# nicolas1805961/Cardiac-Segmentation-Optical-flow

Measured on AMD Instinct MI355X. Metric: cine frames/sec (seg+flow) at 256x256, higher is better.
Workload: dtype f16 MFMA hi/lo split, f32 accumulate (f32-class); 1 GPU; BASELINE config 4: joint seg+flow over 256x256x30 cine slices; Generic_UNet(32 base, 6 pools) 4-flip TTA on every frame + SegFlowGaussian(video.yaml) two-chunk ED-anchored recurrence + fused label warp; image=256x256

## Files before the change

### cardiac-segmentation-optical-flow_amd/cineflow/_lib.py

```python
import ctypes
import os

_HERE = os.path.dirname(os.path.abspath(__file__))
LIB_PATH = os.environ.get("CINEFLOW_LIB") or os.path.join(_HERE, "libcineflow_hip.so")


class CineflowLibraryError(RuntimeError):
    pass


class CineflowError(RuntimeError):
    pass


P = ctypes.c_void_p
I = ctypes.c_int
L = ctypes.c_long
F = ctypes.c_float
DBL = ctypes.c_double

SIGNATURES = {
    "cf_warp_bilinear_2d": [P, P, P, I, I, I, I, P],
    "cf_vecint_2d": [P, P, P, I, I, I, I, P],
    "cf_warp_labels_2d": [P, P, P, I, I, I, I, I, P],
# ... 4 lines not shown
    "cf_corr_volume": [P, P, P, I, I, I, I, I, I, P],
    "cf_corr_volume_route": [P, P, I, I, I, I, I],
    "cf_corr_mfma_enable": [I],
    "cf_corr_pyramid": [P, P, P, I, I, I, I, I, P],
    "cf_corr_lookup": [P, P, P, I, I, I, I, I, P],
    "cf_convex_upsample": [P, P, P, I, I, I, I, P],
    "cf_conv2d": [P, I, P, I, P, L, P, P, P, I, I, I, I, I, I, I, I, I, I, I, I, F, P],
    "cf_conv_transpose2d_k2s2": [P, P, P, P, I, I, I, I, I, I, I, P],
    "cf_conv2d_f16s": [P, I, P, I, P, P, P, P, I, I, I, I, I, I, I, I, I, I, I, I, F, P, I, P],
    "cf_conv3d_f16s": [P, I, P, I, P, P, P, I, I, I, I, I, I, I, I, I, I, F, P, I, P],
    "cf_conv3d_f16s_ok": [I, I, I, I, I, I, I, I, I, I, I],
    "cf_conv3d_pw_f16s": [P, P, P, P, I, I, I, I, I, I, I, I, F, P, I, P],
    "cf_conv3d_pw_f16s_ok": [I, I, I, I, I, I, I, I],
    "cf_conv_transpose2d_k2s2_f16s": [P, P, P, P, I, I, I, I, I, I, I, F, P, I, P],
    "cf_group_norm_apply": [P, P, P, P, P, I, I, I, I, F, I, I, P, P],
    "cf_group_norm_coef": [P, P, P, I, I, I, I, F, P, P],
    "cf_norm_head_1x1": [P, P, F, P, P, P, I, I, I, I, P],
    "cf_batch_norm_coef": [P, P, P, P, F, I, I, P, P],
    "cf_coef_apply_ok": [I, I, L],
    "cf_coef_apply": [P, P, I, F, P, I, I, I, P],
    "cf_conv2d_f16s_prenorm_ok": [I, I, I, I, I],
    "cf_conv_stream_enable": [I],
    "cf_conv2d_f16s_route": [I] * 16 + [P],
    "cf_conv2d_f16s_prenorm": [P, I, P, F, P, P, P, I, I, I, I, F, P, I, P],
    "cf_conv_terms": [I],
    "cf_conv_wino_enable": [I],
    "cf_conv2d_wino_ok": [I, I, I, I, I, I, I],
    "cf_conv2d_wino_form": [I, I, I, I, I, I, I],
    "cf_conv2d_wino_mfma": [I, I, I, I, I, I, I],
    "cf_conv2d_wino": [P, I, P, I, P, P, P, P, I, I, I, I, I, I, I, F, P, I, P],
    "cf_conv2d_wino_prenorm": [P, I, P, F, P, P, P, I, I, I, I, F, P, I, P],
    "cf_group_norm_apply_res_norm": [P, P, P, P, P, I, I, I, I, F, I, I, P, P, P, P, P],
    "cf_group_norm": [P, P, P, P, P, I, I, I, I, F, I, I, P, P],
    "cf_group_norm_stats": [P, P, I, I, I, I, P],
    "cf_group_norm_route": [P, P, P, I, I, I, I, P],
    "cf_layer_norm_cf": [P, P, P, P, I, I, I, F, P],
    "cf_attention_cf": [P, L, P, L, P, L, P, I, I, I, I, I, P],
    "cf_attention_cf_masked": [P, L, P, L, P, L, P, I, I, I, I, I, I, P],
    "cf_attention_cf_route": [P, L, I, I],
    "cf_gru_reset_mul": [P, P, P, I, I, I, P],
    "cf_gru_blend": [P, P, P, P, I, I, I, P],
    "cf_binary": [I, P, P, P, L, L, P],
    "cf_count_out_of_range": [P, L, F, P, P],
    "cf_copy_channels": [P, I, I, P, I, I, I, I, I, I, P],
    "cf_coords_grid": [P, I, I, I, P],
    "cf_crop2d": [P, P, I, I, I, I, I, I, I, P],
# ... 113 lines not shown
```

### cardiac-segmentation-optical-flow_amd/cineflow/ops.py

```python
import collections
import contextlib
import ctypes
import math
import os

import numpy as np
import torch

from ._lib import lib, check

ACT = {None: 0, "none": 0, "gelu": 1, "relu": 2, "lrelu": 3, "tanh": 4, "sigmoid": 5}
ACT_COEF = dict(ACT, mish=6)
RES = {None: 0, "none": 0, "before_act": 1, "after_act": 2}
OP = {"add": 0, "sub": 1, "mul": 2}


def _stream():
    return torch.cuda.current_stream().cuda_stream


def _f32(t, name="tensor"):
    if not isinstance(t, torch.Tensor) or not t.is_cuda:
        raise TypeError("%s must be a CUDA/HIP tensor (cineflow has no CPU path)" % name)
    if t.dtype != torch.float32:
# ... 302 lines not shown
    if res is not None:
        assert res.shape == (B, cout, Ho, Wo)
    assert wpk.dtype == torch.float16 and wpk.is_cuda
    if F16S_RANGE_CHECK:
        _range_check(x1, x2)
    ws, ws_ptr, ws_groups = _stats_args(stats_groups, B, x1.device)
    check(lib().cf_conv2d_f16s(_f32(x1), C1, _opt(x2), C2, wpk.data_ptr(), _opt(bias), _opt(res), _f32(out), out.shape[1], out_coff, B, H, W,
                               cout, kh, kw, stride, pad[0], pad[1], ACT[act], float(alpha) * (2.0 ** -wscale),
                               ws_ptr, ws_groups, _stream()), "cf_conv2d_f16s")
    return (out, ws) if stats_groups else out


F16sRoute = collections.namedtuple("F16sRoute", "route tup terms nimg fused part")


def conv2d_f16s_route(x1, cout, kh, kw, stride=1, pad=(0, 0), x2=None, prenorm=False, transposed=False, stats_groups=None):
    B, C1, H, W = x1.shape
    C2 = 0 if x2 is None else x2.shape[1]
    plan = (ctypes.c_int * 15)()
    route = lib().cf_conv2d_f16s_route(B, C1, C2, H, W, cout, kh, kw, stride, pad[0], pad[1], x1.data_ptr() & 15,
                                       0 if x2 is None else x2.data_ptr() & 15, int(prenorm), int(transposed), stats_groups or 0, plan)
    check(min(route, 0), "cf_conv2d_f16s_route")
    return F16sRoute(route, tuple(plan[1:11]), plan[11], plan[12], bool(plan[13]), plan[14])


def pack_conv3d_weight_f16s(w, c1=None):
    cout, cin, kd, kh, kw = w.shape
    assert (kh, kw) == (3, 3) and kd in (1, 3)
    ntap = kd * 9
    nmt = 1 if cout <= 32 else 2 * ((cout + 63) // 64)
    hi, lo, s, nchunk = _scaled_split(w.reshape(cout, cin, ntap), 16, nmt, c1)
    x = torch.stack([hi, lo]).view(2, nmt, 32, nchunk, 2, 8, ntap)
    return x.permute(1, 3, 6, 0, 4, 2, 5).contiguous().view(-1), s


def conv3d_f16s_ok(B, C1, C2, D, H, W, cout, kernel, stride):
    kernel, stride = tuple(kernel), tuple(stride)
    if kernel[1] != kernel[2] or stride[1] != stride[2]:
        return False
    return lib().cf_conv3d_f16s_ok(B, C1, C2, D, H, W, cout, kernel[0], kernel[1], stride[0], stride[1]) == 1


def conv3d_f16s(x1, wpk, wscale, bias, cout, kernel, stride=(1, 1, 1), x2=None, out=None, alpha=1.0, stats_groups=None):
    B, C1, D, H, W = x1.shape
    C2 = 0 if x2 is None else x2.shape[1]
    kd, kh, kw = kernel
# ... 980 lines not shown
```

### cardiac-segmentation-optical-flow_amd/csrc/conv_f16s.hip

```cpp
#include <hip/hip_fp16.h>
#include <stdlib.h>
#include <string.h>
#include <algorithm>

#include "conv.h"
#include "profile.h"

namespace cf {

typedef float f32x16 __attribute__((ext_vector_type(16)));
typedef _Float16 f16x8 __attribute__((ext_vector_type(8)));

CF_CLOCK_DECL(g_clock_f16s)

struct F16sGeom {
    int TW, TH, NIMG;
    int PH, PW;
    int pstep;
    int ostep;
    int tiles_x, tiles_y, bgroups;
    int nchunk;
    int ablate;
    int c1_pad;
    int NQ;
    int PWR, pwh, kx1, kx2;
    unsigned m_tx, m_ty, m_percg, m_phnq, m_nq, m_nrec, m_phpw, m_pw, m_thtw, m_tw;
};

__host__ __device__ inline unsigned f16s_magic(int d) { return d <= 1 ? 0u : (unsigned)((1ull << 32) / (unsigned)d + 1ull); }
__device__ __forceinline__ int fdiv(int n, int d, unsigned m) { return d <= 1 ? n : (int)__umulhi((unsigned)n, m); }

#ifdef CF_F16S_ABLATION_BUILD
__device__ unsigned long long g_f16s_phase[9];
#define F16S_CLK() __builtin_readcyclecounter()
#endif
template <int KH, int KW, int CK, int WM, int NTW, int MAXT, int NW, int VEC, int PRE, int WL, int TERMS>
__global__ void __launch_bounds__(64 * NW, NW == 8 ? 4 : ((NTW <= 2 && MAXT <= 3) ? 4 : 2))
conv_f16s_kernel(const ConvParams p, const F16sGeom g, const _Float16* __restrict__ wpk) {
    constexpr int KHW = KH * KW;
    constexpr int KS = CK / 16;
    constexpr int REC = CK * 4 + 16;
    constexpr int NT_WG = NTW * (NW / WM);
    constexpr int NG = CK / 8;
    constexpr int NSTAGE = 64 * NW;
    (void)NT_WG;
    extern __shared__ __attribute__((aligned(16))) unsigned char lds[];
    CF_CLOCK_BEGIN();

    const int tid = threadIdx.x;
    const int lane = tid & 63, wave = __builtin_amdgcn_readfirstlane(tid >> 6);
#ifdef CF_F16S_ABLATION_BUILD
    const unsigned long long ph_t0 = F16S_CLK();
    unsigned long long ph_t1 = 0, ph_stage = 0, ph_bar = 0, ph_t2 = 0;
#endif
    const int half = lane >> 5, l31 = lane & 31;
    const int cw = wave % NW;
    const int mt = blockIdx.y * WM + (cw % WM);
    const int ngrp = cw / WM;

// ... 147 lines not shown
                if (!((v_mask[t] >> k) & 1u)) continue;
                f16x4 hi, lo;
                float v[4];
#pragma unroll
                for (int j = 0; j < 4; ++j) {
                    v[j] = stg[t][j][k];
                    if (PRE) {
                        v[j] = (v[j] - cm[j]) * ca[j] + cs[j];
                        v[j] = p.in_slope < 0.f ? gelu_as(v[j]) : (v[j] > 0.f ? v[j] : v[j] * p.in_slope);
                        v[j] = valid ? v[j] : 0.f;
                    }
                }
                split4_f16(v[0], v[1], v[2], v[3], hi, lo);
                *reinterpret_cast<f16x4*>(base + k * REC) = hi;
                *reinterpret_cast<f16x4*>(base + k * REC + CK * 2) = lo;
            }
        }
    };

    float stg0[MAXT][8];
    f32x4v stgv[VT][4];
    if (VEC) issue_loads_v(0, stgv);
    else issue_loads(0, stg0);
    int b_rec[NTW];
#pragma unroll
    for (int nt = 0; nt < NTW; ++nt) {
        int pidx = (ngrp * NTW + nt) * 32 + l31;
        int img = fdiv(pidx, g.TH * g.TW, g.m_thtw);
        int q = pidx - img * (g.TH * g.TW);
        int tyy = fdiv(q, g.TW, g.m_tw), txx = q - tyy * g.TW;
        if (img >= g.NIMG) { img = 0; tyy = 0; txx = 0; }
        b_rec[nt] = ((img * g.PH + tyy * g.ostep) * g.PWR + txx * (g.pwh ? 1 : g.ostep)) * REC + half * 16;
    }

    f32x16 acc1[NTW];
#pragma unroll
    for (int nt = 0; nt < NTW; ++nt)
#pragma unroll
        for (int r = 0; r < 16; ++r) acc1[nt][r] = 0.f;

    constexpr int NSTEP = KHW * KS;
    if constexpr (WL) {
        constexpr int G = (KHW == 9) ? 3 : ((KHW == 1) ? NSTEP : 5);
        constexpr int NGRP = NSTEP / G;
        static_assert(NGRP * G == NSTEP, "weight groups must tile the chunk");
        constexpr int WSLOT = WM * G * 2 * 1024;
// ... 299 lines not shown
                double s1 = 0.0, s2 = 0.0;
                for (int j = 0; j < n; ++j) { s1 += red[2 * (tid + j)]; s2 += red[2 * (tid + j) + 1]; }
                double* w = p.gn_ws + 2L * ((long)b0 * p.gn_groups + co / cpg);
                atomicAdd(w, s1);
                atomicAdd(w + 1, s2);
            }
        }
    }
    CF_CLOCK_END(g_clock_f16s);
#ifdef CF_F16S_ABLATION_BUILD
    if (lane == 0 && ph_t1 && (blockIdx.x & 63) == 5) {
        const unsigned long long t3 = F16S_CLK();
        atomicAdd(&g_f16s_phase[0], ph_t1 - ph_t0);
        atomicAdd(&g_f16s_phase[1], (ph_t2 - ph_t1) - ph_stage - ph_bar);
        atomicAdd(&g_f16s_phase[2], ph_stage);
        atomicAdd(&g_f16s_phase[3], ph_bar);
        atomicAdd(&g_f16s_phase[4], t3 - ph_t2);
        atomicAdd(&g_f16s_phase[5], 1ULL);
        atomicAdd(&g_f16s_phase[6], ph_e1 - ph_t2);
        atomicAdd(&g_f16s_phase[7], ph_e2 - ph_e1);
        atomicAdd(&g_f16s_phase[8], t3 - ph_e2);
    }
#endif
}


static thread_local int t_conv_terms = 3;
int conv_terms() { return t_conv_terms; }

#define CF_F16S_SHAPES(X)                                                                                                                \
     \
    X(3, 3, 16, 1, 1, 2, 8, 1, 0, 1) X(3, 3, 16, 1, 1, 2, 8, 1, 1, 1) X(3, 3, 16, 2, 2, 2, 8, 1, 0, 1) X(3, 3, 16, 2, 2, 2, 8, 1, 1, 1)  \
    X(3, 3, 16, 1, 1, 2, 4, 0, 0, 0) X(3, 3, 16, 1, 1, 2, 4, 1, 0, 0) X(3, 3, 16, 1, 1, 2, 4, 1, 1, 0) X(3, 3, 16, 2, 2, 2, 4, 0, 0, 0)  \
    X(3, 3, 16, 2, 2, 2, 4, 1, 0, 0) X(3, 3, 16, 2, 2, 2, 4, 1, 1, 0) X(3, 3, 16, 4, 4, 2, 4, 0, 0, 0) X(3, 3, 16, 4, 4, 2, 4, 1, 0, 0)  \
    X(3, 3, 16, 4, 4, 2, 4, 1, 1, 0) X(3, 3, 16, 4, 2, 2, 8, 0, 0, 0) X(3, 3, 16, 4, 2, 2, 8, 1, 0, 0)                                   \
                                        \
    X(3, 3, 16, 1, 1, 5, 4, 0, 0, 0) X(3, 3, 16, 2, 1, 3, 4, 0, 0, 0) X(3, 3, 16, 4, 2, 3, 4, 0, 0, 0)                                   \
    X(1, 1, 32, 1, 1, 2, 4, 0, 0, 0) X(1, 1, 32, 2, 2, 2, 4, 0, 0, 0) X(1, 1, 32, 4, 4, 2, 4, 0, 0, 0) X(1, 1, 32, 4, 2, 2, 8, 0, 0, 0)  \
    X(1, 5, 32, 2, 2, 4, 4, 0, 0, 0) X(1, 5, 32, 2, 2, 4, 4, 2, 0, 0) X(1, 5, 32, 4, 2, 4, 8, 0, 0, 0) X(1, 5, 32, 4, 2, 4, 8, 2, 0, 0)  \
    X(5, 1, 32, 2, 2, 4, 4, 0, 0, 0) X(5, 1, 32, 2, 2, 4, 4, 2, 0, 0) X(5, 1, 32, 4, 2, 4, 8, 0, 0, 0) X(5, 1, 32, 4, 2, 4, 8, 2, 0, 0)

struct F16sShape { int KH, KW, CK, WM, NTW, MAXT, NW, VEC, PRE, WL; };
#define CF_F16S_ROW(...) {__VA_ARGS__},
static constexpr F16sShape k_f16s_shapes[] = {CF_F16S_SHAPES(CF_F16S_ROW)};
#undef CF_F16S_ROW

enum { F16S_DECLINED = 0, F16S_KERNEL = 1, F16S_STREAM = 2 };

struct F16sPlan {
    int route = F16S_DECLINED;
    int shape = -1;
    F16sGeom g = {};
    unsigned grid_x = 0, grid_y = 0;
    size_t lds_bytes = 0;
    bool fusable = false;
    const char* why = nullptr;
};
static F16sPlan f16s_declined(const char* why) { F16sPlan pl; pl.why = why; return pl; }

static int f16s_kind(const ConvParams& p) {
    if (p.KH == 3 && p.KW == 3 && p.pad_h == 1 && p.pad_w == 1 && (p.stride == 1 || p.stride == 2)) return 33;
    if (p.KH == 1 && p.KW == 1 && p.pad_h == 0 && p.pad_w == 0 && (p.stride == 1 || p.stride == 2)) return 11;
    if (p.KH == 1 && p.KW == 5 && p.pad_h == 0 && p.pad_w == 2 && p.stride == 1) return 15;
    if (p.KH == 5 && p.KW == 1 && p.pad_h == 2 && p.pad_w == 0 && p.stride == 1) return 51;
    return 0;
}

bool conv_f16s_supported(const ConvParams& p) {
    if (p.w_bstride) return false;
    if (!f16s_kind(p)) return false;
    const long HW = (long)p.H * p.W;
    if ((long)p.C1 * HW * 4 >= (1L << 31) || (long)p.C2 * HW * 4 >= (1L << 31)) return false;
    const double osample = (double)p.out_ctotal * p.Ho * p.Wo * (p.scatter2x2 ? 4.0 : 1.0) * 4.0;
    if (osample * ((long)p.Ho * p.Wo <= 256 ? 8.0 : 1.0) >= 1073741824.0) return false;
// ... 34 lines not shown
    const int NSTAGE = 64 * t.NW;
    const int nrec = g.NIMG * g.PH * g.PW;
    g.m_tx = f16s_magic(g.tiles_x);
    g.m_ty = f16s_magic(g.tiles_y);
    g.m_percg = f16s_magic(g.NIMG * g.PH * g.NQ);
    g.m_phnq = f16s_magic(g.PH * g.NQ);
    g.m_nq = f16s_magic(g.NQ);
    g.m_nrec = f16s_magic(nrec);
    g.m_phpw = f16s_magic(g.PH * g.PW);
    g.m_pw = f16s_magic(g.PW);
    g.m_thtw = f16s_magic(g.TH * g.TW);
    g.m_tw = f16s_magic(g.TW);
    if ((long)g.tiles_x * g.tiles_y * g.bgroups >= (1L << 31) / (g.tiles_x > g.tiles_y ? g.tiles_x : g.tiles_y))
        return f16s_declined("conv_f16s: grid too large for the index decode");
    if (!t.VEC && (nrec * (t.CK / 8) + NSTAGE - 1) / NSTAGE > t.MAXT) return f16s_declined("conv_f16s: staging tasks exceed MAXT");
    pl.fusable = g.NIMG == 1;
    pl.lds_bytes = (size_t)2 * g.NIMG * g.PH * g.PWR * REC + (t.PRE ? (size_t)3 * g.nchunk * t.CK * sizeof(float) : 0) +
                   (t.WL ? (size_t)2 * t.WM * WGRP * 2 * 1024 : 0);
    const size_t stats_lds = (size_t)t.WM * 64 * sizeof(double);
    if (p.gn_ws && pl.fusable && pl.lds_bytes < stats_lds) pl.lds_bytes = stats_lds;
    if ((double)g.NIMG * p.out_ctotal * p.Ho * p.Wo * (p.scatter2x2 ? 4.0 : 1.0) * 4.0 >= 1073741824.0)
        return f16s_declined("conv_f16s: one workgroup's output samples must stay below 1 GiB (32-bit store offsets)");
    if (pl.lds_bytes > 160 * 1024) return f16s_declined("conv_f16s: LDS tile too large");
    pl.route = F16S_KERNEL;
    pl.g = g;
    pl.grid_x = (unsigned)(g.tiles_x * g.tiles_y * g.bgroups), pl.grid_y = (unsigned)((p.Cout + 32 * t.WM - 1) / (32 * t.WM));
    return pl;
}

static F16sPlan f16s_plan(const ConvParams& p) {
    if (conv_stream_applicable(p)) { F16sPlan pl; pl.route = F16S_STREAM; pl.fusable = true; return pl; }
    const int kind = f16s_kind(p);
    const bool k3 = kind == 33, sep = kind == 15 || kind == 51, spatial = k3 || sep;
    const int CK = k3 ? 16 : 32;
    const bool narrow = p.Cout <= 32, s2 = k3 && p.stride == 2;
    bool cout_wide = f16s_cout_wide(p.Cout);
    if (cout_wide && p.Cout % 128 != 0 && !s2) {
        const int tw = std::min(p.Wo, 32), th = std::min(128 / tw, p.Ho);
        const long nwg = (long)((p.Wo + tw - 1) / tw) * ((p.Ho + th - 1) / th) * p.B * ((p.Cout + 127) / 128);
        if (nwg < 1024) cout_wide = false;
    }
    const bool wide = !s2 && cout_wide;
    const int NT_WG = (s2 && !narrow) ? 2 : 4;
    F16sGeom g = {};
    auto geometry = [&](int npx) {
    g.TW = std::min(p.Wo, 32);
// ... 46 lines not shown
        const int nstage = 64 * t.NW, th0 = g.TH;
        while (g.TH > 1 && (g.PH * g.PW * (CK / 8) + nstage - 1) / nstage > t.MAXT) {
            --g.TH;
            g.PH = (g.TH - 1) * p.stride + p.KH;
        }
        if (g.TH != th0) g.tiles_y = (p.Ho + g.TH - 1) / g.TH;
    }
    if (const char* why = f16s_staging(p, t, g)) return f16s_declined(why);
    return f16s_finish(p, t, g);
}

template <int KH, int KW, int CK, int WM, int NTW, int MAXT, int NW, int VEC, int PRE, int WL>
static int launch_f16s_shape(const ConvParams& p, const F16sPlan& pl, const _Float16* wpk, hipStream_t s) {
    F16sGeom g = pl.g;
    size_t lds_bytes = pl.lds_bytes;
#ifdef CF_F16S_ABLATION_BUILD
    { static int ab = -1; if (ab < 0) { const char* e = getenv("CF_F16S_ABLATE"); ab = e ? atoi(e) : 0; } g.ablate = ab; }
    { static long pad = -1; if (pad < 0) { const char* e = getenv("CF_F16S_LDSPAD"); pad = e ? atol(e) : 0; }
      if (pad > (long)lds_bytes) lds_bytes = (size_t)pad; }
    if (lds_bytes > 160 * 1024) { set_error("conv_f16s: LDS tile too large"); return CF_ERR_ARG; }
#endif
    const dim3 grid(pl.grid_x, pl.grid_y), block(64 * NW);
    const double flops = 2.0 * (double)p.B * p.Ho * p.Wo * p.Cout * (p.C1 + p.C2) * p.KH * p.KW;
    if (p.terms == 1)
        return launch_lds<conv_f16s_kernel<KH, KW, CK, WM, NTW, MAXT, NW, VEC, PRE, WL, 1>>("conv_f16s", PK_CONV_F16S, flops, grid, block, lds_bytes, s, p, g, wpk);
    return launch_lds<conv_f16s_kernel<KH, KW, CK, WM, NTW, MAXT, NW, VEC, PRE, WL, 3>>("conv_f16s", PK_CONV_F16S, flops, grid, block, lds_bytes, s, p, g, wpk);
}

#define CF_F16S_ROW(...) launch_f16s_shape<__VA_ARGS__>,
static int (*const k_f16s_launch[])(const ConvParams&, const F16sPlan&, const _Float16*, hipStream_t) = {CF_F16S_SHAPES(CF_F16S_ROW)};
#undef CF_F16S_ROW

static int launch_conv_f16s_part(const ConvParams& p, const _Float16* wpk, hipStream_t s) {
    const F16sPlan pl = f16s_plan(p);
    if (pl.route == F16S_DECLINED) { set_error(pl.why); return CF_ERR_ARG; }
    const bool fused = p.gn_ws && pl.fusable;
    const bool zero = fused && !p.gn_prezeroed;
    const size_t ws_bytes = sizeof(double) * 2 * (size_t)p.B * p.gn_groups;
    if (zero && hipMemsetAsync(p.gn_ws, 0, ws_bytes, s) != hipSuccess) {
        set_error(pl.route == F16S_STREAM ? "conv_stream: memset failed" : "conv_f16s: memset failed");
        return CF_ERR_LAUNCH;
    }
    if (pl.route == F16S_STREAM) return launch_conv_stream(p, wpk, s);
    ConvParams q = p;
    if (!fused) q.gn_ws = nullptr;
    const int rc = k_f16s_launch[pl.shape](q, pl, wpk, s);
// ... 116 lines not shown
    ConvParams p = f16s_layer(B, C, 0, H, W, Cout, 3, 3, 1, 1, 1);
    p.x1 = x; p.bias = bias; p.out = out; p.alpha = alpha; p.in_norm = in_norm; p.in_slope = in_slope;
    f16s_stats(p, gn_ws, gn_groups);
    CF_REQUIRE(!gn_ws || (p.gn_groups > 0 && Cout % p.gn_groups == 0), "bad GroupNorm statistics request");
    CF_REQUIRE(conv_f16s_supported(p), "unsupported configuration for the f16-split kernel");
    return launch_conv_f16s(p, reinterpret_cast<const _Float16*>(wpk), as_stream(stream));
}

extern "C" int cf_conv_transpose2d_k2s2_f16s(const float* x, const void* wpk, const float* bias, float* out, int out_ctotal,
                                             int out_coff, int B, int Cin, int H, int W, int Cout, float alpha, double* gn_ws, int gn_groups,
                                             void* stream) {
    CF_REQUIRE(x && wpk && out, "null pointer");
    CF_REQUIRE(B > 0 && Cin > 0 && H > 0 && W > 0 && Cout > 0, "bad shape");
    CF_REQUIRE(out_coff >= 0 && out_coff + Cout <= out_ctotal, "output channel slice out of range");
    CF_REQUIRE((reinterpret_cast<uintptr_t>(wpk) & 15) == 0, "packed weights must be 16-byte aligned");
    ConvParams p = f16s_layer_transposed(B, Cin, H, W, Cout);
    p.x1 = x; p.bias = bias; p.out = out; p.out_ctotal = out_ctotal; p.out_coff = out_coff; p.alpha = alpha;
    f16s_stats(p, gn_ws, gn_groups);
    CF_REQUIRE(!gn_ws || (p.gn_groups > 0 && Cout % p.gn_groups == 0 && out_coff == 0 && out_ctotal == Cout), "bad GroupNorm statistics request");
    CF_REQUIRE(conv_f16s_supported(p), "unsupported configuration for the f16-split kernel (one sample of the input must stay below 2 GiB)");
    return launch_conv_f16s(p, reinterpret_cast<const _Float16*>(wpk), as_stream(stream));
}

extern "C" int cf_conv2d_f16s_route(int B, int C1, int C2, int H, int W, int Cout, int KH, int KW, int stride, int pad_h, int pad_w, int x1_low4,
                                    int x2_low4, int prenorm, int transposed, int stats_groups, int* plan15) {
    if (plan15) memset(plan15, 0, 15 * sizeof(int));
    CF_REQUIRE(C1 > 0 && C2 >= 0 && B > 0 && H > 0 && W > 0 && Cout > 0 && stride > 0, "bad shape B=%d C=%d+%d H=%d W=%d Cout=%d", B, C1, C2, H, W, Cout);
    CF_REQUIRE(stats_groups >= 0 && (stats_groups == 0 || Cout % stats_groups == 0), "bad GroupNorm statistics request");
    ConvParams p = transposed ? f16s_layer_transposed(B, C1, H, W, Cout) : f16s_layer(B, C1, C2, H, W, Cout, KH, KW, stride, pad_h, pad_w);
    p.x1 = f16s_address(x1_low4);
    if (p.C2) p.x2 = f16s_address(x2_low4);
    if (prenorm && !transposed) { p.in_norm = f16s_address(0); p.in_slope = 0.01f; }
    static double stats;
    if (stats_groups) f16s_stats(p, &stats, stats_groups);
    CF_REQUIRE(p.Ho > 0 && p.Wo > 0, "empty output");
    F16sPlan pl;
    F16sParts parts = {0, 0};
    if (!conv_f16s_supported(p)) {
        pl = f16s_declined(k_f16s_unsupported);
    } else {
        parts = f16s_parts(p);
        p.B = (int)parts.n;
        pl = parts.n < 1 ? f16s_declined("conv_f16s: one sample of the input exceeds 2 GiB") : f16s_plan(p);
    }
    if (pl.route == F16S_DECLINED) { set_error(pl.why); return F16S_DECLINED; }
    if (plan15) {
        const F16sShape t = pl.route == F16S_KERNEL ? k_f16s_shapes[pl.shape] : F16sShape{};
        const int nimg = pl.route == F16S_KERNEL ? pl.g.NIMG : 1;
        const int v[15] = {pl.route, t.KH, t.KW, t.CK, t.WM, t.NTW, t.MAXT, t.NW, t.VEC, t.PRE, t.WL, p.terms, nimg, pl.fusable, (int)parts.n};
        memcpy(plan15, v, sizeof(v));
    }
    return pl.route;
}

#ifdef CF_F16S_ABLATION_BUILD
extern "C" int cf_debug_f16s_phases(unsigned long long* out9) {
    hipDeviceSynchronize();
    hipMemcpyFromSymbol(out9, HIP_SYMBOL(cf::g_f16s_phase), 9 * sizeof(unsigned long long));
    unsigned long long z[9] = {0, 0, 0, 0, 0, 0, 0, 0, 0};
    hipMemcpyToSymbol(HIP_SYMBOL(cf::g_f16s_phase), z, sizeof(z));
    return 0;
}
#endif

namespace cf {
namespace {
__global__ void __launch_bounds__(256) debug_split_kernel(const float* __restrict__ x, unsigned short* __restrict__ hi_old, unsigned short* __restrict__ lo_old,
                                                          unsigned short* __restrict__ hi_new, unsigned short* __restrict__ lo_new, long n) {
    const long npair = n >> 1;
    for (long i = blockIdx.x * (long)blockDim.x + threadIdx.x; i < npair; i += (long)gridDim.x * blockDim.x) {
        const float x0 = x[2 * i], x1 = x[2 * i + 1];
        const _Float16 h0 = (_Float16)x0, h1 = (_Float16)x1;
        const _Float16 l0 = (_Float16)(x0 - (float)h0), l1 = (_Float16)(x1 - (float)h1);
        hi_old[2 * i] = __builtin_bit_cast(unsigned short, h0);
        hi_old[2 * i + 1] = __builtin_bit_cast(unsigned short, h1);
// ... 22 lines not shown
```

### include/cineflow.h

```cpp
#ifndef CINEFLOW_H
#define CINEFLOW_H

#include <stdint.h>

#ifdef __cplusplus
extern "C" {
#endif

#define CF_OK 0
#define CF_ERR_ARG (-1)
#define CF_ERR_LAUNCH (-2)

#define CF_ACT_NONE 0
#define CF_ACT_GELU 1
#define CF_ACT_RELU 2
#define CF_ACT_LRELU 3
#define CF_ACT_TANH 4
#define CF_ACT_SIGMOID 5
#define CF_ACT_MISH 6

#define CF_RES_NONE 0
#define CF_RES_BEFORE_ACT 1
#define CF_RES_AFTER_ACT 2

// ... 52 lines not shown
                  int HW, int groups, float eps, int act, int res_mode, double* ws, void* stream);

int cf_group_norm_apply(const float* x, const float* gamma, const float* beta, const float* res, float* out, int B, int C,
                        int HW, int groups, float eps, int act, int res_mode, const double* ws, void* stream);
int cf_group_norm_stats(const float* x, double* ws, int B, int C, int HW, int groups, void* stream);
int cf_group_norm_route(const float* x, const float* out, const float* res, int B, int C, int HW, int groups, int* plan8);
int cf_group_norm_apply_res_norm(const float* x, const float* gamma, const float* beta, const float* res, float* out, int B, int C,
                                 int HW, int groups, float eps, int act, int res_mode, const double* ws, const double* res_ws,
                                 const float* res_gamma, const float* res_beta, void* stream);
int cf_group_norm_coef(const double* ws, const float* gamma, const float* beta, int B, int C, int HW, int groups, float eps, float* coef,
                       void* stream);
int cf_norm_head_1x1(const float* x, const float* coef, float slope, const float* w, const float* bias, float* out, int B, int C, int HW,
                     int K, void* stream);
int cf_batch_norm_coef(const float* running_mean, const float* running_var, const float* gamma, const float* beta, float eps, int B, int C,
                       float* coef, void* stream);
int cf_coef_apply_ok(int B, int C, long HW);
int cf_coef_apply(const float* x, const float* coef, int act, float slope, float* out, int B, int C, int HW, void* stream);
int cf_conv_stream_enable(int on);
int cf_conv2d_f16s_prenorm_ok(int B, int C, int H, int W, int Cout);
int cf_conv2d_f16s_prenorm(const float* x, int C, const float* in_norm, float in_slope, const void* wpk, const float* bias, float* out,
                           int B, int H, int W, int Cout, float alpha, double* gn_ws, int gn_groups, void* stream);
int cf_conv2d_f16s_route(int B, int C1, int C2, int H, int W, int Cout, int KH, int KW, int stride, int pad_h, int pad_w, int x1_low4,
                         int x2_low4, int prenorm, int transposed, int stats_groups, int* plan15);

int cf_conv2d_wino_ok(int B, int C1, int C2, int H, int W, int Cout, int prenorm);
int cf_conv2d_wino_form(int B, int C1, int C2, int H, int W, int Cout, int prenorm);
int cf_conv2d_wino_mfma(int B, int C1, int C2, int H, int W, int Cout, int prenorm);
int cf_conv_wino_enable(int level);
int cf_conv2d_wino(const float* x1, int C1, const float* x2, int C2, const void* wpk, const float* bias, const float* res, float* out,
                   int out_ctotal, int out_coff, int B, int H, int W, int Cout, int act, float alpha, double* gn_ws, int gn_groups,
                   void* stream);
int cf_conv2d_wino_prenorm(const float* x, int C, const float* in_norm, float in_slope, const void* wpk, const float* bias, float* out,
                           int B, int H, int W, int Cout, float alpha, double* gn_ws, int gn_groups, void* stream);

int cf_layer_norm_cf(const float* x, const float* gamma, const float* beta, float* out, int B, int C, int N, float eps,
                     void* stream);

int cf_attention_cf(const float* q, long q_bs, const float* k, long k_bs, const float* v, long v_bs, float* out, int B,
                    int heads, int d, int Nq, int Nk, void* stream);
int cf_attention_cf_masked(const float* q, long q_bs, const float* k, long k_bs, const float* v, long v_bs, float* out, int B,
                           int heads, int d, int Nq, int Nk, int nk_valid, void* stream);
int cf_attention_cf_route(const float* v, long v_bs, int d, int Nk);

int cf_gru_reset_mul(const float* gates, const float* h, float* rh, int B, int C, int HW, void* stream);
int cf_gru_blend(const float* gates, const float* h, const float* cand, float* out, int B, int C, int HW, void* stream);

// ... 145 lines not shown
```

Before: 832.5 frames/s.

## Add 16x16x32 MFMA path for split-f16 3x3 stride-1 convolutions

Adds a second form of the hi/lo split f16 conv kernel that uses the 16x16x32 f16 MFMA instruction. It packs tap pairs across lane groups and handles the odd ninth tap by masking half the lanes. The form has its own LDS weight ring and a register-prefetch weight path, a vectorised output store and a GroupNorm statistics epilogue. It is enabled by default (env level 1) for two built 3x3 stride-1 shapes, aiming for higher MFMA throughput per issued instruction on the dominant UNet convs. The cost is extra register pressure, wasted lanes on the leftover tap, and a large new code path that adds correctness risk.

```diff
diff --git a/cardiac-segmentation-optical-flow_amd/cineflow/_lib.py b/cardiac-segmentation-optical-flow_amd/cineflow/_lib.py
--- a/cardiac-segmentation-optical-flow_amd/cineflow/_lib.py
+++ b/cardiac-segmentation-optical-flow_amd/cineflow/_lib.py
@@ -50,6 +50,8 @@
     "cf_conv2d_f16s_prenorm_ok": [I, I, I, I, I],
     "cf_conv_stream_enable": [I],
     "cf_conv2d_f16s_route": [I] * 16 + [P],
+    "cf_conv2d_f16s_mfma": [I] * 16,
+    "cf_conv_f16s_mfma_enable": [I],
     "cf_conv2d_f16s_prenorm": [P, I, P, F, P, P, P, I, I, I, I, F, P, I, P],
     "cf_conv_terms": [I],
     "cf_conv_wino_enable": [I],
diff --git a/cardiac-segmentation-optical-flow_amd/cineflow/ops.py b/cardiac-segmentation-optical-flow_amd/cineflow/ops.py
--- a/cardiac-segmentation-optical-flow_amd/cineflow/ops.py
+++ b/cardiac-segmentation-optical-flow_amd/cineflow/ops.py
@@ -348,6 +348,17 @@
                                        0 if x2 is None else x2.data_ptr() & 15, int(prenorm), int(transposed), stats_groups or 0, plan)
     check(min(route, 0), "cf_conv2d_f16s_route")
     return F16sRoute(route, tuple(plan[1:11]), plan[11], plan[12], bool(plan[13]), plan[14])
+
+
+def conv2d_f16s_mfma(x1, cout, kh, kw, stride=1, pad=(0, 0), x2=None, prenorm=False, transposed=False, stats_groups=None):
+    B, C1, H, W = x1.shape
+    C2 = 0 if x2 is None else x2.shape[1]
+    return int(lib().cf_conv2d_f16s_mfma(B, C1, C2, H, W, cout, kh, kw, stride, pad[0], pad[1], x1.data_ptr() & 15,
+                                         0 if x2 is None else x2.data_ptr() & 15, int(prenorm), int(transposed), stats_groups or 0))
+
+
+def conv_f16s_mfma_enable(level):
+    return int(lib().cf_conv_f16s_mfma_enable(int(level)))
 
 
 def pack_conv3d_weight_f16s(w, c1=None):
diff --git a/cardiac-segmentation-optical-flow_amd/csrc/conv_f16s.hip b/cardiac-segmentation-optical-flow_amd/csrc/conv_f16s.hip
--- a/cardiac-segmentation-optical-flow_amd/csrc/conv_f16s.hip
+++ b/cardiac-segmentation-optical-flow_amd/csrc/conv_f16s.hip
@@ -23,18 +23,27 @@
     int ablate;
     int c1_pad;
     int NQ;
+    int vec4;
     int PWR, pwh, kx1, kx2;
     unsigned m_tx, m_ty, m_percg, m_phnq, m_nq, m_nrec, m_phpw, m_pw, m_thtw, m_tw;
 };
 
 __host__ __device__ inline unsigned f16s_magic(int d) { return d <= 1 ? 0u : (unsigned)((1ull << 32) / (unsigned)d + 1ull); }
 __device__ __forceinline__ int fdiv(int n, int d, unsigned m) { return d <= 1 ? n : (int)__umulhi((unsigned)n, m); }
+__device__ __forceinline__ f16x8 lane_select(bool c, f16x8 a, f16x8 b) {
+    typedef unsigned u32x4 __attribute__((ext_vector_type(4)));
+    const u32x4 ua = __builtin_bit_cast(u32x4, a), ub = __builtin_bit_cast(u32x4, b);
+    u32x4 r;
+#pragma unroll
+    for (int k = 0; k < 4; ++k) r[k] = c ? ua[k] : ub[k];
+    return __builtin_bit_cast(f16x8, r);
+}
 
 #ifdef CF_F16S_ABLATION_BUILD
 __device__ unsigned long long g_f16s_phase[9];
 #define F16S_CLK() __builtin_readcyclecounter()
 #endif
-template <int KH, int KW, int CK, int WM, int NTW, int MAXT, int NW, int VEC, int PRE, int WL, int TERMS>
+template <int KH, int KW, int CK, int WM, int NTW, int MAXT, int NW, int VEC, int PRE, int WL, int TERMS, int M16 = 0>
 __global__ void __launch_bounds__(64 * NW, NW == 8 ? 4 : ((NTW <= 2 && MAXT <= 3) ? 4 : 2))
 conv_f16s_kernel(const ConvParams p, const F16sGeom g, const _Float16* __restrict__ wpk) {
     constexpr int KHW = KH * KW;
@@ -228,6 +237,349 @@
     f32x4v stgv[VT][4];
     if (VEC) issue_loads_v(0, stgv);
     else issue_loads(0, stg0);
+    if constexpr (M16) {
+        static_assert(TERMS == 3 && KHW == 9 && CK == 16, "the 16x16x32 form is built for the split products of 3x3 layers");
+        typedef unsigned u32x4 __attribute__((ext_vector_type(4)));
+        constexpr int NSTEP = KHW * KS;
+        const int l15 = lane & 15, kg = lane >> 4;
+        f16x8 nxh, nxl;
+        int x_rec[NTW][2];
+#pragma unroll
+        for (int nt = 0; nt < NTW; ++nt)
+#pragma unroll
+            for (int pb = 0; pb < 2; ++pb) {
+                int pidx = (ngrp * NTW + nt) * 32 + pb * 16 + l15;
+                int img = fdiv(pidx, g.TH * g.TW, g.m_thtw);
+                int q = pidx - img * (g.TH * g.TW);
+                int tyy = fdiv(q, g.TW, g.m_tw), txx = q - tyy * g.TW;
+                if (img >= g.NIMG) { img = 0; tyy = 0; txx = 0; }
+                x_rec[nt][pb] = ((img * g.PH + tyy * g.ostep) * g.PWR + txx * (g.pwh ? 1 : g.ostep)) * REC + (kg & 1) * 16;
+                asm volatile("" : "+v"(x_rec[nt][pb]));
+            }
+        auto tap_off = [&](int tap) {
+            const int ky = tap / KW, kx = tap % KW;
+            return (ky * g.PWR + (g.pwh ? (kx >> 1) + (kx & 1) * g.pwh : kx)) * REC;
+        };
+        auto pair_off = [&](int j) { return (kg >> 1) ? tap_off(2 * j + 1) : tap_off(2 * j); };
+
+        f32x4v acc[NTW][2][2];
+#pragma unroll
+        for (int nt = 0; nt < NTW; ++nt)
+#pragma unroll
+            for (int pb = 0; pb < 2; ++pb)
+#pragma unroll
+                for (int cb = 0; cb < 2; ++cb) acc[nt][pb][cb] = f32x4v{0.f, 0.f, 0.f, 0.f};
+
+        auto x_load = [&](const unsigned char* xb, int nt, int pb, int off) __attribute__((always_inline)) {
+            const unsigned char* rp = xb + x_rec[nt][pb] + off;
+            nxh = *reinterpret_cast<const f16x8*>(rp);
+            nxl = *reinterpret_cast<const f16x8*>(rp + CK * 2);
+        };
+        auto nothing = []() {};
+        auto mfma_group = [&](const unsigned char* xb, int off, int off_next, const f16x8 (&wh)[2], const f16x8 (&wl_)[2], const bool left,
+                              auto before_last) __attribute__((always_inline)) {
+#pragma unroll
+            for (int blk = 0; blk < 2 * NTW; ++blk) {
+                const int nt = blk >> 1, pb = blk & 1;
+                const f16x8 xh = nxh, xl = left ? lane_select(kg < 2, nxl, f16x8{}) : nxl;
+                if (blk + 1 < 2 * NTW) x_load(xb, (blk + 1) >> 1, (blk + 1) & 1, off);
+                else if (off_next >= 0) x_load(xb, 0, 0, off_next);
+                if (blk + 1 == 2 * NTW) before_last();
+                __builtin_amdgcn_sched_barrier(0);
+#pragma unroll
+                for (int q = left ? 1 : 0; q < 3; ++q)
+#pragma unroll
+                    for (int cb = 0; cb < 2; ++cb)
+                        acc[nt][pb][cb] = __builtin_amdgcn_mfma_f32_16x16x32_f16(q == 1 ? xl : xh, q == 0 ? wl_[cb] : wh[cb], acc[nt][pb][cb], 0, 0, 0);
+            }
+        };
+        auto fill_ctab = [&]() {
+            float* ct = reinterpret_cast<float*>(lds + 2 * buf_bytes);
+            for (int k = tid; k < 3 * ctab_n; k += 64 * NW) {
+                const int which = k / ctab_n, c = k - which * ctab_n;
+                ct[k] = c < p.C1 ? p.in_norm[((long)b0 * 3 + which) * p.C1 + c] : 0.f;
+            }
+            __syncthreads();
+        };
+
+        if constexpr (WL) {
+            static_assert(KHW == 9, "the LDS weight ring of this form holds kernel rows");
+            constexpr int G = 3, NGRP = 3;
+            constexpr int WSLOT = WM * G * 2 * 1024;
+            unsigned char* wl = lds + 2 * buf_bytes + (PRE ? 3 * ctab_n * 4 : 0);
+            const f16x8* wbase = reinterpret_cast<const f16x8*>(wpk) + lane;
+            const int nq = g.nchunk * NGRP;
+            auto issue_w = [&](int q) {
+                const unsigned dst0 = (unsigned)(size_t)((__attribute__((address_space(3))) unsigned char*)(wl + (q & 1) * WSLOT));
+                for (int f = wave; f < WM * G * 2; f += NW) {
+                    const int m = f / (G * 2), j = f - m * (G * 2);
+                    const f16x8* src = wbase + (((long)(blockIdx.y * WM + m) * g.nchunk * NSTEP + (long)q * G) * 2 + j) * 64;
+                    const unsigned dst = __builtin_amdgcn_readfirstlane(dst0 + (unsigned)f * 1024u);
+                    unsigned keep;
+                    asm volatile("s_mov_b32 %0, m0\n\ts_mov_b32 m0, %2\n\ts_nop 0\n\tglobal_load_lds_dwordx4 %1, off\n\ts_mov_b32 m0, %0"
+                                 : "=&s"(keep) : "v"(src), "s"(dst) : "memory");
+                }
+            };
+            issue_w(0);
+            if (PRE) fill_ctab();
+            if (VEC) write_stage_v(0, stgv);
+            else write_stage(0, stg0);
+            asm volatile("s_waitcnt vmcnt(0)" ::: "memory");
+            __syncthreads();
+            const unsigned char* wa = wl + ((cw % WM) * G * 2) * 1024 + ((kg & 1) * 32 + l15) * 16;
+            const int wq_pair = (kg >> 1) * 2048, wq_left = (kg >> 1) * 1024;
+            auto read_w = [&](const unsigned char* ws, int sg, int lane_off, f16x8 (&wh)[2], f16x8 (&wl_)[2]) __attribute__((always_inline)) {
+#pragma unroll
+                for (int cb = 0; cb < 2; ++cb) {
+                    wh[cb] = *reinterpret_cast<const f16x8*>(ws + lane_off + (sg * 2) * 1024 + cb * 256);
+                    wl_[cb] = *reinterpret_cast<const f16x8*>(ws + lane_off + (sg * 2 + 1) * 1024 + cb * 256);
+                }
+            };
+            for (int c = 0; c < g.nchunk; ++c) {
+                const bool more = c + 1 < g.nchunk;
+                const unsigned char* xb = lds + (c & 1) * buf_bytes;
+                f16x8 ch[2], cl[2];
+                x_load(xb, 0, 0, pair_off(0));
+#pragma unroll
+                for (int grp = 0; grp < NGRP; ++grp) {
+                    const int q = c * NGRP + grp;
+                    if (q + 1 < nq) issue_w(q + 1);
+                    if (grp == 0) {
+                        const int cn = more ? c + 1 : c;
+                        if (VEC) issue_loads_v(cn, stgv);
+                        else issue_loads(cn, stg0);
+                    }
+                    __builtin_amdgcn_sched_barrier(0);
+                    const unsigned char* ws = wa + (q & 1) * WSLOT;
+                    f16x8 wh[2], wl_[2];
+                    if (grp == 0) {
+                        read_w(ws, 0, wq_pair, wh, wl_);
+                        read_w(ws, 2, 0, ch, cl);
+                        mfma_group(xb, pair_off(0), pair_off(1), wh, wl_, false, nothing);
+                        asm volatile("s_waitcnt lgkmcnt(0)" ::: "memory");
+                    } else if (grp == 1) {
+                        read_w(ws, 0, 0, wh, wl_);
+#pragma unroll
+                        for (int cb = 0; cb < 2; ++cb) {
+                            wh[cb] = lane_select(kg < 2, ch[cb], wh[cb]);
+                            wl_[cb] = lane_select(kg < 2, cl[cb], wl_[cb]);
+                        }
+                        mfma_group(xb, pair_off(1), pair_off(2), wh, wl_, false, nothing);
+                        read_w(ws, 1, wq_pair, wh, wl_);
+                        mfma_group(xb, pair_off(2), pair_off(3), wh, wl_, false, nothing);
+                    } else {
+                        read_w(ws, 0, wq_pair, wh, wl_);
+                        f16x8 wm[2];
+                        mfma_group(xb, pair_off(3), tap_off(8), wh, wl_, false, [&]() {
+#pragma unroll
+                            for (int cb = 0; cb < 2; ++cb) wm[cb] = *reinterpret_cast<const f16x8*>(ws + wq_left + 4 * 1024 + cb * 256);
+                        });
+                        mfma_group(xb, tap_off(8), -1, wm, wm, true, nothing);
+                    }
+                    if (grp == NGRP - 1 && more) {
+                        if (VEC) write_stage_v(c + 1, stgv);
+                        else write_stage(c + 1, stg0);
+                    }
+                    if (VEC && grp == 0 && NGRP > 1) asm volatile("s_waitcnt vmcnt(%0)" :: "n"(VEC * 4) : "memory");
+                    else asm volatile("s_waitcnt vmcnt(0)" ::: "memory");
+                    __syncthreads();
+                }
+            }
+        } else {
+            constexpr int NPAIR = 4;
+            const f16x8* wfrag = reinterpret_cast<const f16x8*>(wpk) + (long)mt * g.nchunk * (NSTEP * 2) * 64 + (kg & 1) * 32 + l15;
+            const f16x8* wpair = wfrag + (kg >> 1) * 128;
+            const f16x8* wleft = wfrag + (kg >> 1) * 64;
+            f16x8 wH[2][2] = {}, wL[2][2] = {}, wM[2] = {};
+            auto load_pair = [&](int chunk, int j, int slot) {
+                const f16x8* wc = wpair + ((long)chunk * NSTEP + 2 * j) * 128;
+#pragma unroll
+                for (int cb = 0; cb < 2; ++cb) {
+                    wH[slot][cb] = wc[cb * 16];
+                    wL[slot][cb] = wc[64 + cb * 16];
+                }
+            };
+            auto load_left = [&](int chunk) {
+                const f16x8* wc = wleft + ((long)chunk * NSTEP + 8) * 128;
+#pragma unroll
+                for (int cb = 0; cb < 2; ++cb) wM[cb] = wc[cb * 16];
+            };
+            load_pair(0, 0, 0);
+            if (PRE) fill_ctab();
+            if (VEC) write_stage_v(0, stgv);
+            else write_stage(0, stg0);
+            __syncthreads();
+            for (int c = 0; c < g.nchunk; ++c) {
+                const bool more = c + 1 < g.nchunk;
+                const int cn = more ? c + 1 : c;
+                const unsigned char* xb = lds + (c & 1) * buf_bytes;
+                x_load(xb, 0, 0, pair_off(0));
+#pragma unroll
+                for (int j = 0; j < NPAIR; ++j) {
+                    if (j + 1 < NPAIR) load_pair(c, j + 1, (j + 1) & 1);
+                    else load_left(c);
+                    if (j == 0) {
+                        if (VEC) issue_loads_v(cn, stgv);
+                        else issue_loads(cn, stg0);
+                    }
+                    __builtin_amdgcn_sched_barrier(0);
+                    mfma_group(xb, pair_off(j), j + 1 < NPAIR ? pair_off(j + 1) : tap_off(8), wH[j & 1], wL[j & 1], false, nothing);
+                }
+                load_pair(cn, 0, 0);
+                __builtin_amdgcn_sched_barrier(0);
+                mfma_group(xb, tap_off(8), -1, wM, wM, true, nothing);
+                if (more) {
+                    if (VEC) write_stage_v(c + 1, stgv);
+                    else write_stage(c + 1, stg0);
+                }
+                __syncthreads();
+            }
+        }
+
+        bool co_ok[2];
+        unsigned ochan[2];
+        constexpr unsigned OOB_PX = 0x80000000u, OOB_CH = 0x40000000u;
+#pragma unroll
+        for (int cb = 0; cb < 2; ++cb) {
+            const int co = mt * 32 + cb * 16 + l15;
+            co_ok[cb] = co < p.Cout;
+            ochan[cb] = co_ok[cb] ? (unsigned)co * (unsigned)HoWo * 4u : OOB_CH;
+            float bv = 0.f;
+            if (p.bias && co_ok[cb]) bv = p.bias[co];
+#pragma unroll
+            for (int nt = 0; nt < NTW; ++nt)
+#pragma unroll
+                for (int pb = 0; pb < 2; ++pb)
+#pragma unroll
+                    for (int r = 0; r < 4; ++r) acc[nt][pb][cb][r] = p.alpha * acc[nt][pb][cb][r] + bv;
+        }
+        auto act_all = [&](const int a) __attribute__((always_inline)) {
+#pragma unroll
+            for (int nt = 0; nt < NTW; ++nt)
+#pragma unroll
+                for (int pb = 0; pb < 2; ++pb)
+#pragma unroll
+                    for (int cb = 0; cb < 2; ++cb)
+#pragma unroll
+                        for (int r = 0; r < 4; ++r) {
+                            acc[nt][pb][cb][r] = act_apply(acc[nt][pb][cb][r], a);
+                            __builtin_amdgcn_sched_barrier(0);
+                        }
+        };
+        switch (p.act) {
+            case CF_ACT_GELU: act_all(CF_ACT_GELU); break;
+            case CF_ACT_RELU: act_all(CF_ACT_RELU); break;
+            case CF_ACT_LRELU: act_all(CF_ACT_LRELU); break;
+            case CF_ACT_TANH: act_all(CF_ACT_TANH); break;
+            case CF_ACT_SIGMOID: act_all(CF_ACT_SIGMOID); break;
+            default: break;
+        }
+        const unsigned osample = (unsigned)p.out_ctotal * (unsigned)HoWo;
+        const __amdgpu_buffer_rsrc_t rs_out = __builtin_amdgcn_make_buffer_rsrc(
+            p.out + ((long)b0 * p.out_ctotal + p.out_coff) * (long)HoWo, 0,
+            (int)(((unsigned)(b0 + g.NIMG <= p.B ? g.NIMG : p.B - b0) * osample - (unsigned)p.out_coff * (unsigned)HoWo) * 4u), 0x00020000);
+        auto px_decode = [&](int pidx, bool& ok, unsigned& off, long& roff) __attribute__((always_inline)) {
+            asm volatile("" : "+v"(pidx));
+            int img = fdiv(pidx, g.TH * g.TW, g.m_thtw);
+            const int q = pidx - img * (g.TH * g.TW);
+            int tyy = fdiv(q, g.TW, g.m_tw), txx = q - tyy * g.TW;
+            const bool in_tile = img < g.NIMG;
+            if (!in_tile) { img = 0; tyy = 0; txx = 0; }
+            const int b = b0 + img, oy = y0 + tyy, ox = x0 + txx;
+            ok = in_tile && b < p.B && oy < p.Ho && ox < p.Wo;
+            off = ok ? ((unsigned)img * osample + (unsigned)oy * p.Wo + ox) * 4u : OOB_PX;
+            roff = (long)b * p.Cout * HoWo + (long)oy * p.Wo + ox;
+        };
+        float ssum[2] = {0.f, 0.f}, ssq[2] = {0.f, 0.f};
+#pragma unroll
+        for (int nt = 0; nt < NTW; ++nt)
+#pragma unroll
+            for (int pb = 0; pb < 2; ++pb) {
+                const int pbase = (ngrp * NTW + nt) * 32 + pb * 16 + 4 * kg;
+                if (g.vec4) {
+                    bool ok;
+                    unsigned off;
+                    long roff;
+                    px_decode(pbase, ok, off, roff);
+#pragma unroll
+                    for (int cb = 0; cb < 2; ++cb) {
+                        f32x4v v = acc[nt][pb][cb];
+                        const bool okc = ok && co_ok[cb];
+                        if (p.res) {
+                            if (okc) {
+                                const float* rp = p.res + roff + (long)(mt * 32 + cb * 16 + l15) * HoWo;
+#pragma unroll
+                                for (int r = 0; r < 4; ++r) v[r] += rp[r];
+                            }
+                        }
+                        __builtin_amdgcn_raw_buffer_store_b128(__builtin_bit_cast(u32x4, v), rs_out, off + ochan[cb], 0, 0);
+#pragma unroll
+                        for (int r = 0; r < 4; ++r) {
+                            const float m = okc ? v[r] : 0.f;
+                            ssum[cb] += m;
+                            ssq[cb] += m * m;
+                        }
+                    }
+                } else {
+#pragma unroll
+                    for (int r = 0; r < 4; ++r) {
+                        bool ok;
+                        unsigned off;
+                        long roff;
+                        px_decode(pbase + r, ok, off, roff);
+#pragma unroll
+                        for (int cb = 0; cb < 2; ++cb) {
+                            float v = acc[nt][pb][cb][r];
+                            const bool okc = ok && co_ok[cb];
+                            if (p.res) { if (okc) v += p.res[roff + (long)(mt * 32 + cb * 16 + l15) * HoWo]; }
+                            __builtin_amdgcn_raw_buffer_store_b32(__builtin_bit_cast(unsigned, v), rs_out, off + ochan[cb], 0, 0);
+                            const float m = okc ? v : 0.f;
+                            ssum[cb] += m;
+                            ssq[cb] += m * m;
+                        }
+                    }
+                }
+            }
+        if (do_stats) {
+#pragma unroll
+            for (int cb = 0; cb < 2; ++cb) {
+                ssum[cb] += __shfl_xor(ssum[cb], 16, 64);
+                ssum[cb] += __shfl_xor(ssum[cb], 32, 64);
+                ssq[cb] += __shfl_xor(ssq[cb], 16, 64);
+                ssq[cb] += __shfl_xor(ssq[cb], 32, 64);
+            }
+            double* red = reinterpret_cast<double*>(lds);
+            __syncthreads();
+            if (tid < WM * 64) red[tid] = 0.0;
+            __syncthreads();
+            if (kg == 0) {
+#pragma unroll
+                for (int cb = 0; cb < 2; ++cb) {
+                    const int cl = (cw % WM) * 32 + cb * 16 + l15;
+                    atomicAdd(&red[2 * cl], (double)ssum[cb]);
+                    atomicAdd(&red[2 * cl + 1], (double)ssq[cb]);
+                }
+            }
+            __syncthreads();
+            if (tid < WM * 32 && b0 < p.B) {
+                const int cbase = blockIdx.y * WM * 32;
+                const int co = cbase + tid;
+                const int cpg = p.Cout / p.gn_groups;
+                if (co < p.Cout && (tid == 0 || co % cpg == 0)) {
+                    int n = cpg - co % cpg;
+                    if (n > WM * 32 - tid) n = WM * 32 - tid;
+                    if (n > p.Cout - co) n = p.Cout - co;
+                    double s1 = 0.0, s2 = 0.0;
+                    for (int j = 0; j < n; ++j) { s1 += red[2 * (tid + j)]; s2 += red[2 * (tid + j) + 1]; }
+                    double* w = p.gn_ws + 2L * ((long)b0 * p.gn_groups + co / cpg);
+                    atomicAdd(w, s1);
+                    atomicAdd(w + 1, s2);
+                }
+            }
+        }
+        CF_CLOCK_END(g_clock_f16s);
+        return;
+    } else {
     int b_rec[NTW];
 #pragma unroll
     for (int nt = 0; nt < NTW; ++nt) {
@@ -573,6 +925,7 @@
         atomicAdd(&g_f16s_phase[8], t3 - ph_e2);
     }
 #endif
+    }
 }
 
 
@@ -594,13 +947,40 @@
 struct F16sShape { int KH, KW, CK, WM, NTW, MAXT, NW, VEC, PRE, WL; };
 #define CF_F16S_ROW(...) {__VA_ARGS__},
 static constexpr F16sShape k_f16s_shapes[] = {CF_F16S_SHAPES(CF_F16S_ROW)};
+
+#define CF_F16S_M16_SHAPES(X) \
+    X(3, 3, 16, 2, 2, 2, 8, 1, 1, 1) X(3, 3, 16, 4, 2, 2, 8, 1, 0, 0)
+static constexpr F16sShape k_f16s_m16_shapes[] = {CF_F16S_M16_SHAPES(CF_F16S_ROW)};
 #undef CF_F16S_ROW
+static constexpr bool f16s_m16_built(const F16sShape& t) {
+    for (const F16sShape& s : k_f16s_m16_shapes)
+        if (s.KH == t.KH && s.KW == t.KW && s.CK == t.CK && s.WM == t.WM && s.NTW == t.NTW && s.MAXT == t.MAXT && s.NW == t.NW && s.VEC == t.VEC &&
+            s.PRE == t.PRE && s.WL == t.WL)
+            return true;
+    return false;
+}
+
+static int g_f16s_mfma_level = -1;
+static int f16s_mfma_level() {
+    if (g_f16s_mfma_level < 0) {
+        const char* e = getenv("CF_CONV_F16S_MFMA");
+        const int v = e ? atoi(e) : 1;
+        g_f16s_mfma_level = (v == 0 || v == 1 || v == 16) ? v : 1;
+    }
+    return g_f16s_mfma_level;
+}
+
+static bool f16s_m16_class(bool k3, int stride, bool deferred, bool wl) {
+    if (!k3 || stride != 1) return false;
+    return wl ? deferred : !deferred;
+}
 
 enum { F16S_DECLINED = 0, F16S_KERNEL = 1, F16S_STREAM = 2 };
 
 struct F16sPlan {
     int route = F16S_DECLINED;
     int shape = -1;
+    int mfma = 32;
     F16sGeom g = {};
     unsigned grid_x = 0, grid_y = 0;
     size_t lds_bytes = 0;
@@ -681,6 +1061,10 @@
     if ((double)g.NIMG * p.out_ctotal * p.Ho * p.Wo * (p.scatter2x2 ? 4.0 : 1.0) * 4.0 >= 1073741824.0)
         return f16s_declined("conv_f16s: one workgroup's output samples must stay below 1 GiB (32-bit store offsets)");
     if (pl.lds_bytes > 160 * 1024) return f16s_declined("conv_f16s: LDS tile too large");
+    const int lvl = f16s_mfma_level();
+    const bool can16 = f16s_m16_built(t) && p.terms == 3 && !p.scatter2x2;
+    if (can16 && (lvl == 16 || (lvl == 1 && f16s_m16_class(t.KH == 3, p.stride, t.PRE != 0, t.WL != 0)))) pl.mfma = 16;
+    g.vec4 = (g.TW & 3) == 0 && (p.Wo & 3) == 0 && (reinterpret_cast<uintptr_t>(p.out) & 15) == 0;
     pl.route = F16S_KERNEL;
     pl.g = g;
     pl.grid_x = (unsigned)(g.tiles_x * g.tiles_y * g.bgroups), pl.grid_y = (unsigned)((p.Cout + 32 * t.WM - 1) / (32 * t.WM));
@@ -773,6 +1157,9 @@
 #endif
     const dim3 grid(pl.grid_x, pl.grid_y), block(64 * NW);
     const double flops = 2.0 * (double)p.B * p.Ho * p.Wo * p.Cout * (p.C1 + p.C2) * p.KH * p.KW;
+    if constexpr (f16s_m16_built(F16sShape{KH, KW, CK, WM, NTW, MAXT, NW, VEC, PRE, WL}))
+        if (pl.mfma == 16)
+            return launch_lds<conv_f16s_kernel<KH, KW, CK, WM, NTW, MAXT, NW, VEC, PRE, WL, 3, 1>>("conv_f16s", PK_CONV_F16S, flops, grid, block, lds_bytes, s, p, g, wpk);
     if (p.terms == 1)
         return launch_lds<conv_f16s_kernel<KH, KW, CK, WM, NTW, MAXT, NW, VEC, PRE, WL, 1>>("conv_f16s", PK_CONV_F16S, flops, grid, block, lds_bytes, s, p, g, wpk);
     return launch_lds<conv_f16s_kernel<KH, KW, CK, WM, NTW, MAXT, NW, VEC, PRE, WL, 3>>("conv_f16s", PK_CONV_F16S, flops, grid, block, lds_bytes, s, p, g, wpk);
@@ -935,9 +1322,10 @@
     return launch_conv_f16s(p, reinterpret_cast<const _Float16*>(wpk), as_stream(stream));
 }
 
-extern "C" int cf_conv2d_f16s_route(int B, int C1, int C2, int H, int W, int Cout, int KH, int KW, int stride, int pad_h, int pad_w, int x1_low4,
-                                    int x2_low4, int prenorm, int transposed, int stats_groups, int* plan15) {
+static int f16s_route_query(int B, int C1, int C2, int H, int W, int Cout, int KH, int KW, int stride, int pad_h, int pad_w, int x1_low4,
+                            int x2_low4, int prenorm, int transposed, int stats_groups, int* plan15, int* mfma) {
     if (plan15) memset(plan15, 0, 15 * sizeof(int));
+    if (mfma) *mfma = 0;
     CF_REQUIRE(C1 > 0 && C2 >= 0 && B > 0 && H > 0 && W > 0 && Cout > 0 && stride > 0, "bad shape B=%d C=%d+%d H=%d W=%d Cout=%d", B, C1, C2, H, W, Cout);
     CF_REQUIRE(stats_groups >= 0 && (stats_groups == 0 || Cout % stats_groups == 0), "bad GroupNorm statistics request");
     ConvParams p = transposed ? f16s_layer_transposed(B, C1, H, W, Cout) : f16s_layer(B, C1, C2, H, W, Cout, KH, KW, stride, pad_h, pad_w);
@@ -963,7 +1351,26 @@
         const int v[15] = {pl.route, t.KH, t.KW, t.CK, t.WM, t.NTW, t.MAXT, t.NW, t.VEC, t.PRE, t.WL, p.terms, nimg, pl.fusable, (int)parts.n};
         memcpy(plan15, v, sizeof(v));
     }
+    if (mfma && pl.route == F16S_KERNEL) *mfma = pl.mfma;
     return pl.route;
+}
+
+extern "C" int cf_conv2d_f16s_route(int B, int C1, int C2, int H, int W, int Cout, int KH, int KW, int stride, int pad_h, int pad_w, int x1_low4,
+                                    int x2_low4, int prenorm, int transposed, int stats_groups, int* plan15) {
+    return f16s_route_query(B, C1, C2, H, W, Cout, KH, KW, stride, pad_h, pad_w, x1_low4, x2_low4, prenorm, transposed, stats_groups, plan15, nullptr);
+}
+
+extern "C" int cf_conv2d_f16s_mfma(int B, int C1, int C2, int H, int W, int Cout, int KH, int KW, int stride, int pad_h, int pad_w, int x1_low4,
+                                   int x2_low4, int prenorm, int transposed, int stats_groups) {
+    int mfma = 0;
+    f16s_route_query(B, C1, C2, H, W, Cout, KH, KW, stride, pad_h, pad_w, x1_low4, x2_low4, prenorm, transposed, stats_groups, nullptr, &mfma);
+    return mfma;
+}
+
+extern "C" int cf_conv_f16s_mfma_enable(int level) {
+    const int prev = f16s_mfma_level();
+    if (level == 0 || level == 1 || level == 16) g_f16s_mfma_level = level;
+    return prev;
 }
 
 #ifdef CF_F16S_ABLATION_BUILD
diff --git a/include/cineflow.h b/include/cineflow.h
--- a/include/cineflow.h
+++ b/include/cineflow.h
@@ -98,6 +98,9 @@
                            int B, int H, int W, int Cout, float alpha, double* gn_ws, int gn_groups, void* stream);
 int cf_conv2d_f16s_route(int B, int C1, int C2, int H, int W, int Cout, int KH, int KW, int stride, int pad_h, int pad_w, int x1_low4,
                          int x2_low4, int prenorm, int transposed, int stats_groups, int* plan15);
+int cf_conv2d_f16s_mfma(int B, int C1, int C2, int H, int W, int Cout, int KH, int KW, int stride, int pad_h, int pad_w, int x1_low4,
+                        int x2_low4, int prenorm, int transposed, int stats_groups);
+int cf_conv_f16s_mfma_enable(int level);
 
 int cf_conv2d_wino_ok(int B, int C1, int C2, int H, int W, int Cout, int prenorm);
 int cf_conv2d_wino_form(int B, int C1, int C2, int H, int W, int Cout, int prenorm);
```

New measurement: 834.8 frames/s, median of 6. About the same (+0.3%).
